# alexpreynolds/starch3

Hardware: AMD Instinct MI355X
Metric: input BED MB/s (cfg2, bzip2 -9, archive bit-identical to CPU starch3 path) (higher is better)
Workload: dtype u8

## Files before the change

starch_amd/csrc/bz2_bwt3.hip:

```cpp
#include "bz2_int.hpp"
#include "bz2_bwt.hpp"

#include <stdio.h>
#include <string.h>

#include <algorithm>
#include <type_traits>
#include <vector>

namespace bz {
namespace {

constexpr int PT = 256;
constexpr int PTILE = 32768;
constexpr int PDIG = 12;
constexpr int PNB = 1 << PDIG;
constexpr int PNB_WIDE = 8192;
static_assert(PTILE <= 32768 && PNB_WIDE <= 8192, "k3_scatter_lds packs (digit << 15) | rotation-in-tile");
constexpr int MAXT = (900064 + PTILE - 1) / PTILE;
constexpr uint32_t W_MAX = 64, S1_MAX = 128, S_MAX = 256, M0_MAX = 512, M1_MAX = 1024, M2_MAX = 2048, M3_MAX = 4096;
#ifndef STARCH_L_MIN
#define STARCH_L_MIN 4096
#endif
constexpr uint32_t L_MIN = STARCH_L_MIN;
// ... 76 lines not shown
    BwtScratch scr;
    Lists L;
    uint32_t nb;
    uint32_t lsel;
    uint32_t tsel;
    uint32_t mode;
    uint32_t keysrc;
    uint64_t* kA;
    uint64_t* kB;
    uint8_t* lA;
    uint8_t* lB;
    uint32_t rtext;
    uint32_t* qhead;
    const uint32_t* qseg;
    uint32_t nbins;
    uint32_t sdig;
};

__device__ __forceinline__ int bits_for3(uint32_t x) { return x ? 32 - __clz(x) : 0; }

__device__ __forceinline__ void wave_sync_lds3()
{
    __builtin_amdgcn_fence(__ATOMIC_RELEASE, "wavefront");
    __builtin_amdgcn_wave_barrier();
    __builtin_amdgcn_fence(__ATOMIC_ACQUIRE, "wavefront");
}

__device__ __forceinline__ uint64_t lanemask_lt()
{
    const int lane = threadIdx.x & 63;
    return lane ? (~0ull >> (64 - lane)) : 0ull;
}

#ifndef STARCH_NT
#define STARCH_NT 0
#endif
#ifndef STARCH_W_UNROLL
#define STARCH_W_UNROLL 0
#endif
template <class T>
__device__ __forceinline__ T ld_nt(const T* p)
{
    if constexpr (STARCH_NT != 0) return __builtin_nontemporal_load(p);
    else return *p;
}
template <class T>
__device__ __forceinline__ void st_nt(T* p, T v)
{
    if constexpr (STARCH_NT != 0) __builtin_nontemporal_store(v, p);
    else *p = v;
}

__device__ __forceinline__ void wave_push(uint32_t* ctr, uint64_t* list, bool pred, uint64_t item)
{
    const uint64_t m = __ballot(pred);
    if (!m) return;
    const int leader = __ffsll((unsigned long long)m) - 1;
    const int lane = threadIdx.x & 63;
    uint32_t base = 0;
    if (lane == leader) base = atomicAdd(ctr, (uint32_t)__popcll(m));
    base = __shfl(base, leader, 64);
    if (pred) list[base + __popcll(m & lanemask_lt())] = item;
}

__device__ __forceinline__ int size_class(uint32_t m)
{
    return m <= W_MAX ? 0 : m <= S1_MAX ? 1 : m <= S_MAX ? 2 : m > L_MIN ? 6 : m <= M0_MAX ? 7 : m <= M1_MAX ? 3 : m <= M2_MAX ? 4
         : m <= M3_MAX ? 5 : 6;
}
__device__ __forceinline__ uint64_t* class_list(const Ctx& c, int cls)
{
    return cls == 0 ? c.L.w : cls == 1 ? c.L.s : cls == 2 ? c.L.s2 : cls == 3 ? c.L.m1 : cls == 4 ? c.L.m2
         : cls == 5 ? c.L.m3 : cls == 7 ? c.L.m0 : c.L.l[c.lsel];
}
__device__ __forceinline__ uint32_t* class_ctr(const Ctx& c, int cls)
{
    return c.L.ctr + (cls == 0 ? C_W : cls == 1 ? C_S : cls == 2 ? C_S2 : cls == 3 ? C_M1 : cls == 4 ? C_M2
                      : cls == 5 ? C_M3 : cls == 7 ? C_M0 : C_L0 + c.lsel);
}

__device__ __forceinline__ void wg_classify(const Ctx& c, uint32_t* sh, bool pred, uint32_t slot, uint32_t s,
                                            uint32_t m, uint32_t shift, uint32_t par)
{
    const int cls = pred ? size_class(m) : -1;
// ... 354 lines not shown
                    const uint64_t a = ix == 0 ? w[0] : ix == 1 ? w[1] : w[2];
                    const uint64_t nx = ix == 0 ? w[1] : ix == 1 ? w[2] : w[3];
                    d[u] = top_digit((a << pb) | ((nx >> 1) >> (63u - pb)), geo);
                }
            }
#pragma unroll
            for (int u = 0; u < SU; ++u) {
                const uint32_t q = q0 + u;
                p[u] = q < e ? atomicAdd(&cur[d[u]], 1u) : 0u;
            }
#pragma unroll
            for (int u = 0; u < SU; ++u) {
                const uint32_t q = q0 + u;
                if (q < e) {
                    const uint32_t r = t0 + q;
                    SA[p[u]] = r;
                    if (tot[d[u]] == 1u) {
                        c.scr.LL[so + p[u]] = (uint8_t)pss_bits(pss, (uint64_t)(r ? r - 1u : n - 1u) * B, B);
                        if (r == 0) c.blocks[b].orig_ptr = p[u];
                    }
                }
            }
        }
        __syncthreads();
    }
}

template <int NB, bool MAT>
__global__ void __launch_bounds__(SCT) k3_scatter_lds(Ctx c)
{
    constexpr uint32_t SH_HALF = NB == PNB ? PTILE / 2 : PTILE / 4;
    constexpr int SU = (int)(SH_HALF / SCT);
    constexpr int BPT = NB / SCT;
    __shared__ uint32_t cur[NB], tot[NB], lst[NB + 1];
    __shared__ uint32_t stage[SH_HALF];
    __shared__ uint8_t stage8[MAT ? 4 : SH_HALF];
    __shared__ uint32_t scan_sh[SCT / 64 + 1];
    __shared__ uint32_t qs[8];
    __shared__ uint32_t job_sh;
    constexpr uint32_t PWN = MAT ? (SH_HALF + 1) * 8 / 64 + 4 : 1;
    __shared__ uint64_t pw[PWN];
    constexpr bool mat = MAT;
    const int tid = threadIdx.x;
    const uint32_t x = xcc_id();
    if (tid < 8) qs[tid] = ((uint32_t)tid < c.nb ? (c.nb - tid + 7) / 8 : 0u) * MAXT;
    __syncthreads();
    for (;;) {
        const uint32_t job = wg_pop(c, qs, &job_sh, x);
        if (job == 0xFFFFFFFFu) break;
        const uint32_t y = job >> 28, k = job & 0x0FFFFFFFu;
        const uint32_t slot = y + 8u * (k / MAXT), tile = k % MAXT;
        const uint32_t b = c.b0 + slot;
        const uint32_t n = c.blocks[b].n;
        const uint32_t t0 = tile * PTILE;
        if (t0 >= n) continue;
        const uint64_t so = (uint64_t)slot * c.scr.stride;
        const uint32_t* th = tile_hist(c, slot);
        for (int i = tid; i < NB; i += SCT) { cur[i] = th[(uint64_t)tile * NB + i]; tot[i] = th[(uint64_t)MAXT * NB + i]; }
        const Geo geo = c.L.geo[slot];
        const uint32_t B = geo.B;
        const uint64_t* pss = c.scr.K + so;
        uint32_t* SA = c.scr.SA + so;
        uint64_t* KM = c.kA + so;
        uint8_t* LS = c.lA ? c.lA + so : nullptr;
        const uint32_t e = n - t0 < (uint32_t)PTILE ? n - t0 : (uint32_t)PTILE;
        for (uint32_t h0 = 0; h0 < e; h0 += SH_HALF) {
            const uint32_t he = e - h0 < SH_HALF ? e - h0 : SH_HALF;
            for (int i = tid; i < NB; i += SCT) lst[i] = 0;
            const uint32_t rs = t0 + h0;
            const uint64_t wbase = rs ? ((uint64_t)(rs - 1) * B) >> 6 : 0;
            if constexpr (mat) {
                const uint64_t wend = (((uint64_t)(rs + he) * B + 64) >> 6) + 2;
                for (uint64_t w = wbase + tid; w < wend; w += SCT) pw[w - wbase] = pss[w];
            }
            __syncthreads();
            const uint32_t q0 = tid * SU;
            uint32_t d[SU], p[SU];
            uint8_t sd[SU];
            {
                const uint64_t bit0 = (uint64_t)(t0 + h0 + q0) * B;
                const uint64_t qw = bit0 >> 6;
                const uint32_t p0 = (uint32_t)(bit0 & 63u);
                const uint64_t w[4] = {pss[qw], pss[qw + 1], pss[qw + 2], pss[qw + 3]};
                const uint32_t sds = 64u - geo.SH - 8u;
#pragma unroll
                for (int u = 0; u < SU; ++u) {
                    const uint32_t bit = p0 + (uint32_t)u * B;
                    const uint32_t ix = bit >> 6, pb = bit & 63u;
                    const uint64_t a = ix == 0 ? w[0] : ix == 1 ? w[1] : w[2];
                    const uint64_t nx = ix == 0 ? w[1] : ix == 1 ? w[2] : w[3];
                    const uint64_t v = (a << pb) | ((nx >> 1) >> (63u - pb));
                    d[u] = top_digit(v, geo);
                    sd[u] = (uint8_t)(v >> sds);
                }
            }
#pragma unroll
            for (int u = 0; u < SU; ++u) p[u] = (q0 + u < he) ? atomicAdd(&lst[d[u]], 1u) : 0u;
            __syncthreads();
            {
                uint32_t v[BPT], sum = 0;
#pragma unroll
                for (int q = 0; q < BPT; ++q) { v[q] = lst[tid * BPT + q]; sum += v[q]; }
                uint32_t run = block_excl_scan_add<uint32_t>(sum, scan_sh, (uint32_t*)nullptr);
#pragma unroll
                for (int q = 0; q < BPT; ++q) { lst[tid * BPT + q] = run; run += v[q]; }
                if (tid == SCT - 1) lst[NB] = run;
            }
            __syncthreads();
#pragma unroll
            for (int u = 0; u < SU; ++u)
                if (q0 + u < he) {
                    const uint32_t j = lst[d[u]] + p[u];
                    stage[j] = (d[u] << 15) | (h0 + q0 + u);
                    if constexpr (!MAT) stage8[j] = sd[u];
                }
            __syncthreads();
            for (uint32_t j = tid; j < he; j += SCT) {
                const uint32_t v = stage[j];
                const uint32_t dg = v >> 15, r = t0 + (v & 0x7FFFu);
                const uint32_t pos = cur[dg] + (j - lst[dg]);
                st_nt(SA + pos, r);
                uint32_t ls = 0;
                if (mat && r) {
                    const uint64_t bit = (uint64_t)(r - 1) * B - (wbase << 6);
                    const uint32_t q = (uint32_t)(bit >> 6), p = (uint32_t)(bit & 63u);
                    ls = (uint32_t)(((pw[q] << p) | ((pw[q + 1] >> 1) >> (63u - p))) >> (64u - B));
                } else if (mat || tot[dg] == 1u) {
                    ls = (uint32_t)pss_bits(pss, (uint64_t)(r ? r - 1u : n - 1u) * B, B);
                }
                if (mat) {
                    const uint64_t bit = (uint64_t)r * B - (wbase << 6);
                    const uint32_t q = (uint32_t)(bit >> 6), p = (uint32_t)(bit & 63u);
                    KM[pos] = ((pw[q] << p) | ((pw[q + 1] >> 1) >> (63u - p))) >> (64u - geo.KB);
                    LS[pos] = (uint8_t)ls;
                }
                if (tot[dg] == 1u) {
                    c.scr.LL[so + pos] = (uint8_t)ls;
                    if (r == 0) c.blocks[b].orig_ptr = pos;
                } else if (!mat && tot[dg] > L_MIN) {
                    c.scr.LL[so + pos] = stage8[j];
                }
            }
            __syncthreads();
            for (int i = tid; i < NB; i += SCT) cur[i] += lst[i + 1] - lst[i];
            __syncthreads();
        }
    }
}

constexpr uint32_t BIN_CH = 4096;
constexpr uint32_t BIN_MAXWG = 128;

__device__ __forceinline__ uint32_t bin_of(uint64_t it, uint32_t i, uint32_t vs)
{
    return (it_slot(it) << vs) | ((i >> 6) & ((1u << vs) - 1u));
}

__global__ void __launch_bounds__(256) k3_bin_hist(const uint64_t* __restrict__ in, uint32_t n, uint32_t nb,
                                                    uint32_t ch, uint32_t* __restrict__ hist,
                                                    uint32_t* __restrict__ colsum, uint32_t vs)
{
    __shared__ uint32_t h[4096];
    for (uint32_t i = threadIdx.x; i < nb; i += 256) h[i] = 0;
    __syncthreads();
    const uint32_t a = blockIdx.x * ch, e = a + ch < n ? a + ch : n;
    for (uint32_t i0 = a; i0 < e; i0 += 256) {
        const uint32_t i = i0 + threadIdx.x;
        const bool ok = i < e;
        const uint32_t b = ok ? bin_of(in[i], i, vs) : 0u;
        const uint64_t act = __ballot(ok);
        if (!act) continue;
        const int lead = __ffsll((unsigned long long)act) - 1;
        const uint32_t b0 = (uint32_t)__shfl((int)b, lead, 64);
        if (__ballot(ok && b == b0) == act) {
            if ((int)(threadIdx.x & 63) == lead) atomicAdd(&h[b0], (uint32_t)__popcll(act));
        } else if (ok) {
            atomicAdd(&h[b], 1u);
        }
    }
// ... 123 lines not shown
        uint8_t* dl = DBL && ks.l ? (par ? c.lA : c.lB) + base : nullptr;
        uint32_t* SA = c.scr.SA + base;
        uint32_t* RK = c.scr.RK + so;
        const uint32_t db = shift < 8 ? shift : 8;
        const uint32_t sh2 = shift - db;
        const uint64_t dmask = (1ull << db) - 1ull;
        const uint8_t* sdig = nullptr;
        if (!DBL && c.sdig && c.rtext == 0 && !c.mode && par == 0 && db == 8) {
            const Geo g = c.L.geo[slot];
            if (shift == g.KB - g.SH) sdig = c.scr.LL + base;
        }
        for (int i = tid; i < LW * 256; i += LT) (&wh[0][0])[i] = 0;
        if (tid == 0) big[256] = 0;
        __syncthreads();
        PLT(t1);
        PLA(0, t0, t1);
#ifndef STARCH_PART_PU
#define STARCH_PART_PU 24
#endif
        constexpr int PU = STARCH_PART_PU;
        for (uint32_t i0 = 0; i0 < m; i0 += PU * LT) {
            uint32_t d[PU];
            if (sdig) {
#pragma unroll
                for (int u = 0; u < PU; ++u) {
                    const uint32_t i = i0 + u * LT + tid;
                    d[u] = sdig[i < m ? i : 0u];
                }
            } else {
                uint32_t vv[PU];
#pragma unroll
                for (int u = 0; u < PU; ++u) {
                    const uint32_t i = i0 + u * LT + tid;
                    vv[u] = ld_nt(sv + (i < m ? i : 0u));
                }
#pragma unroll
                for (int u = 0; u < PU; ++u) {
                    const uint32_t i = i0 + u * LT + tid;
                    d[u] = (uint32_t)((elem_key<DBL>(ks, s + (i < m ? i : 0u), vv[u]) >> sh2) & dmask);
                }
            }
#pragma unroll
            for (int u = 0; u < PU; ++u) {
                const uint32_t i = i0 + u * LT + tid;
                if (!DBL && m <= PL_CAP && i < m) dcache[i] = (uint8_t)d[u];
            }
#pragma unroll
            for (int u = 0; u < PU; ++u)
                if (i0 + u * LT + tid < m) atomicAdd(&wh[wid][d[u]], 1u);
        }
        __syncthreads();
        PLT(t2);
        PLA(1, t1, t2);
        uint32_t tcount = 0;
        if (tid < 256) for (int w = 0; w < LW; ++w) tcount += wh[w][tid];
        const uint32_t pre = block_excl_scan_add<uint32_t>(tid < 256 ? tcount : 0u, scan_sh, (uint32_t*)nullptr);
        if (tid < 256) { st[tid] = pre; cur[tid] = pre; cntd[tid] = tcount; }
        __syncthreads();
        PLT(t3);
        PLA(2, t2, t3);
        const bool staged = !DBL && m <= PL_STG && !(STARCH_PL_STG == 0);
        for (uint32_t i0 = 0; i0 < m; i0 += PU * LT) {
            uint32_t v[PU];
            uint64_t k[PU];
            uint8_t lsy[PU];
#pragma unroll
            for (int u = 0; u < PU; ++u) {
                const uint32_t i = i0 + u * LT + tid;
                v[u] = ld_nt(sv + (i < m ? i : 0u));
            }
            if (!DBL && m <= PL_CAP) {
#pragma unroll
                for (int u = 0; u < PU; ++u) {
                    const uint32_t i = i0 + u * LT + tid;
                    k[u] = (uint64_t)dcache[i < m ? i : 0u] << sh2;
                }
            } else if (sdig) {
#pragma unroll
                for (int u = 0; u < PU; ++u) {
                    const uint32_t i = i0 + u * LT + tid;
                    k[u] = (uint64_t)sdig[i < m ? i : 0u] << sh2;
                }
            } else {
#pragma unroll
                for (int u = 0; u < PU; ++u) {
                    const uint32_t i = i0 + u * LT + tid;
                    k[u] = elem_key<DBL>(ks, s + (i < m ? i : 0u), v[u]);
                }
            }
#pragma unroll
            for (int u = 0; u < PU; ++u) {
                const uint32_t i = i0 + u * LT + tid;
                lsy[u] = dl ? ks.l[s + (i < m ? i : 0u)] : (uint8_t)0;
            }
#pragma unroll
            for (int u = 0; u < PU; ++u) {
                if (i0 + u * LT + tid < m) {
                    const uint32_t p = atomicAdd(&cur[(uint32_t)((k[u] >> sh2) & dmask)], 1u);
                    if (!DBL && staged) stg[p] = v[u];
                    else st_nt(dv + p, v[u]);
                    if constexpr (DBL) dk[p] = k[u];
                    if (dl) dl[p] = lsy[u];
                }
            }
        }
        __syncthreads();
        if (!DBL && staged) {
            for (uint32_t i = tid; i < m; i += LT) st_nt(dv + i, stg[i]);
            __syncthreads();
        }
        PLT(t4);
        PLA(3, t3, t4);
        uint32_t nruns = 0;
        if (tid < 256) {
            const uint32_t cc = cntd[tid], ss = st[tid];
            if (cc == 1) {
                const uint32_t v = dv[ss];
                if (!par) SA[ss] = v;
                c.scr.LL[base + ss] = dl ? dl[ss] : last_sym(c, slot, v);
                if (c.mode) RK[v] = s + ss;
                if (v == 0) c.blocks[b].orig_ptr = s + ss;
                nruns = 1;
            } else if (size_class(cc) == 6 && sh2 == 0) {
                big[atomicAdd(&big[256], 1u)] = tid;
                nruns = 1;
            }
        }
        {
            const uint32_t cc = tid < 256 ? cntd[tid] : 0u;
            const bool push = tid < 256 && cc >= 2 && !(size_class(cc) == 6 && sh2 == 0);
            wg_classify(c, cls_sh, push, slot, s + (tid < 256 ? st[tid] : 0u), cc, sh2, par ^ 1u);
        }
        if (tid < 256) {
            const uint32_t r = wave_reduce_add(nruns);
            if (c.mode && (tid & 63) == 0 && r) atomicAdd(&c.L.runs[slot], r);
        }
        __syncthreads();
        PLT(t5);
        PLA(4, t4, t5);
        const uint32_t nbig = big[256];
        for (uint32_t q = 0; q < nbig; ++q) {
// ... 461 lines not shown
        const uint32_t* info = c.L.hg_info + (uint64_t)q * 512;
        const uint32_t st = info[tid] & ~HG_FINAL;
        const uint32_t en = tid < 255 ? (info[tid + 1] & ~HG_FINAL) : g.m;
        const uint32_t fsz = (info[tid] & HG_FINAL) ? en - st : 0u;
        uint32_t ftot = 0;
        const uint32_t fp = block_excl_scan_add<uint32_t>(fsz, scan_sh, &ftot);
        fin_pre[tid] = fp;
        if (tid == 255) fin_pre[256] = ftot;
        __syncthreads();
        for (uint32_t x = slice * 256u + tid; x < ftot; x += per * 256u) {
            uint32_t lo = 0, hi = 255;
            while (lo < hi) {
                const uint32_t mid = (lo + hi + 1) >> 1;
                if (fin_pre[mid] <= x) lo = mid; else hi = mid - 1;
            }
            const uint32_t b0 = info[lo] & ~HG_FINAL;
            const uint32_t p = b0 + (x - fin_pre[lo]);
            const uint32_t v = dv[p];
            if (!g.par) c.scr.SA[base + p] = v;
            const uint32_t be = lo < 255 ? (info[lo + 1] & ~HG_FINAL) : g.m;
            if (be - b0 == 1) c.scr.LL[base + p] = dl ? dl[p] : last_sym(c, g.slot, v);
            if (c.mode) c.scr.RK[so + v] = g.s + b0;
            if (v == 0) c.blocks[c.b0 + g.slot].orig_ptr = g.s + p;
        }
        __syncthreads();
    }
}

__device__ __forceinline__ void emit_sorted(const Ctx& c, uint32_t slot, uint32_t s, uint32_t j, uint32_t v,
                                            bool valid, uint32_t hp, bool end, uint32_t& runs_acc, uint32_t lsym)
{
    const uint64_t so = (uint64_t)slot * c.scr.stride;
    if (valid) {
        st_nt(c.scr.SA + so + s + j, v);
        st_nt(c.scr.LL + so + s + j, (uint8_t)lsym);
        if (c.mode) c.scr.RK[so + v] = s + hp;
        if (v == 0) c.blocks[c.b0 + slot].orig_ptr = s + j;
    }
    const bool tie = valid && end && j > hp;
    const uint64_t tb = __ballot(tie);
    if (tb) {
        wave_push(c.L.ctr + C_T0 + c.tsel, c.L.t[c.tsel], tie, mk_item(slot, s + hp, j - hp + 1, 0, 0));
        const uint32_t te = wave_reduce_add<uint32_t>(tie ? j - hp + 1 : 0u);
        if ((threadIdx.x & 63) == 0) atomicAdd(c.L.ctr + C_TS0 + c.tsel, te);
    }
    runs_acc += (uint32_t)__popcll(__ballot(valid && end));
}

__device__ __forceinline__ void emit_vals(const Ctx& c, uint32_t slot, uint32_t s, uint32_t j, uint32_t v, bool valid,
                                          uint32_t hp, uint32_t lsym)
{
    if (valid) {
        const uint64_t so = (uint64_t)slot * c.scr.stride;
        st_nt(c.scr.SA + so + s + j, v);
        st_nt(c.scr.LL + so + s + j, (uint8_t)lsym);
        if (c.mode) c.scr.RK[so + v] = s + hp;
        if (v == 0) c.blocks[c.b0 + slot].orig_ptr = s + j;
    }
}

template <int NW>
__device__ __forceinline__ uint32_t tie_reserve(const Ctx& c, uint32_t tcnt, uint32_t* tc, int wid, int lane)
{
    uint32_t* ctr = c.L.ctr + C_T0 + c.tsel;
    if constexpr (NW == 1) {
        uint32_t base = 0;
        if (lane == 0 && tcnt) base = atomicAdd(ctr, tcnt);
        return (uint32_t)__shfl((int)base, 0, 64);
    } else {
        if (lane == 0) tc[wid] = tcnt;
        __syncthreads();
        if (wid == 0 && lane == 0) {
            uint32_t t = 0;
#pragma unroll
            for (int w = 0; w < NW; ++w) t += tc[w];
            tc[NW] = t ? atomicAdd(ctr, t) : 0u;
        }
        __syncthreads();
        uint32_t base = tc[NW];
        for (int w = 0; w < wid; ++w) base += tc[w];
        return base;
    }
}

__device__ __forceinline__ uint64_t shfl64(uint64_t v, uint32_t src)
{
    const uint32_t lo = (uint32_t)__shfl((int)(uint32_t)v, (int)src, 64);
    const uint32_t hi = (uint32_t)__shfl((int)(uint32_t)(v >> 32), (int)src, 64);
// ... 16 lines not shown

template <bool DBL>
__global__ void __launch_bounds__(256) k3_sort_w(Ctx c, const uint64_t* __restrict__ items)
{
    __shared__ uint64_t skey[4][W_MAX + 1];
    __shared__ uint32_t sval[4][W_MAX];
    const uint32_t lane = threadIdx.x & 63, wid = threadIdx.x >> 6;
    const uint32_t xs8 = blockIdx.x & 7u, wseg = (gridDim.x >> 3) * 4u, w_in = (blockIdx.x >> 3) * 4u + wid;
    const uint32_t seg0 = c.qseg[xs8], seg1 = c.qseg[xs8 + 1];
    const uint32_t per_w = (seg1 - seg0 + wseg - 1) / wseg;
    const uint32_t ch = per_w >= 64u ? 64u : (per_w ? per_w : 1u);
    for (uint32_t cb = seg0 + w_in * ch; cb < seg1; cb += wseg * ch) {
        const uint32_t cnt = seg1 - cb < ch ? seg1 - cb : ch;
        const uint64_t myitem = lane < cnt ? items[cb + lane] : 0ull;
        const uint32_t msz = lane < cnt ? it_size(myitem) : 0u;
        for (uint32_t done = 0; done < cnt;) {
            const uint32_t sz = (lane >= done && lane < cnt) ? msz : 0u;
            const uint32_t incl = wave_incl_scan_add(sz);
            const bool take = lane >= done && lane < cnt && incl <= 64u;
            const uint32_t ng = (uint32_t)__popcll(__ballot(take));
            const uint32_t off = incl - sz;
            const uint32_t total = (uint32_t)__shfl((int)incl, (int)(done + ng - 1), 64);
            const uint64_t smask = wave_reduce_or64(take ? (1ull << off) : 0ull);
            const bool valid = lane < total;
            const uint64_t upto = lane == 63 ? ~0ull : ((2ull << lane) - 1ull);
            const uint32_t gi = valid ? done + (uint32_t)__popcll(smask & upto) - 1u : done;
            const uint64_t item = shfl64(myitem, gi);
            const uint32_t goff = (uint32_t)__shfl((int)off, (int)gi, 64);
            const uint32_t gstart = valid ? goff : 0u;
            const uint32_t slot = it_slot(item), s = it_start(item), m = it_size(item), par = it_par(item);
            const uint32_t j = valid ? lane - gstart : 0u;
            const uint32_t* sv = (par ? c.scr.V : c.scr.SA) + (uint64_t)slot * c.scr.stride + s;
            const KeySrc ks = key_src(c, slot, par);
            const uint32_t v = ld_nt(sv + j);
            uint32_t ls;
            uint64_t k = elem_key<DBL>(c, ks, slot, s + j, v, ls);
            if (!valid) k = ~0ull;
            uint32_t r = 0;
            if (ng == 1) {
#if STARCH_W_UNROLL
#pragma unroll 4
#endif
                for (uint32_t q = 0; q < total; ++q) {
                    const uint64_t kq = ((uint64_t)(uint32_t)__builtin_amdgcn_readlane((int)(k >> 32), (int)q) << 32) |
                                        (uint32_t)__builtin_amdgcn_readlane((int)(uint32_t)k, (int)q);
                    r += (kq < k || (kq == k && q < j)) ? 1u : 0u;
                }
            } else {
                const uint32_t maxm = wave_reduce_max(valid ? m : 0u);
#if STARCH_W_UNROLL
#pragma unroll 4
#endif
                for (uint32_t q = 0; q < maxm; ++q) {
                    const bool in = valid && q < m;
                    const uint64_t kq = shfl64(k, in ? gstart + q : lane);
                    r += (in && (kq < k || (kq == k && q < j))) ? 1u : 0u;
                }
            }
            wave_sync_lds3();
            if (valid) { skey[wid][gstart + r] = k; sval[wid][gstart + r] = v | (ls << 24); }
            wave_sync_lds3();
            const uint64_t key = valid ? skey[wid][lane] : 0;
            const uint32_t val = valid ? sval[wid][lane] : 0;
            const bool head = valid && (j == 0 || skey[wid][lane - 1] != key);
            const bool end = valid && (j + 1 == m || skey[wid][lane + 1] != key);
            const uint32_t hp = wave_incl_scan_max<uint32_t>(head ? lane : 0u) - gstart;
            asm volatile("s_waitcnt vmcnt(0)" ::: "memory");
// ... 37 lines not shown

template <int NW>
__device__ __forceinline__ void gsync()
{
    if constexpr (NW == 1) wave_sync_lds3();
    else __syncthreads();
}

template <int E>
struct GrpIn {
    uint64_t item;
    KeySrc ks;
    uint32_t v[E];
    uint32_t v0;
    uint64_t kx[E];
    uint32_t ls[E];
    uint64_t k0;
    uint64_t kb[E];
    uint32_t lb[E];
    uint64_t k0b;
    bool one;
};

template <int NW, int E>
__device__ __forceinline__ void grp_load_vals(const Ctx& c, GrpIn<E>& x, bool ok, int wid, int lane)
{
    if (!ok) x.item = mk_item(0, 0, 1, 0, 0);
    const uint32_t slot = it_slot(x.item), s = it_start(x.item), m = it_size(x.item), par = it_par(x.item);
    const uint32_t* sv = (par ? c.scr.V : c.scr.SA) + (uint64_t)slot * c.scr.stride + s;
    x.ks = key_src(c, slot, par);
#pragma unroll
    for (int e = 0; e < E; ++e) {
        const uint32_t i = (uint32_t)(wid * 64 * E + e * 64 + lane);
        x.v[e] = ld_nt(sv + (i < m ? i : 0u));
    }
    x.v0 = sv[0];
}

__device__ __forceinline__ uint32_t pss_rr(const KeySrc& ks, uint32_t r)
{
    const uint32_t rr = r + ks.off;
    return rr >= ks.n ? rr - ks.n : rr;
}
__device__ __forceinline__ uint32_t pss_pr(const KeySrc& ks, uint32_t r) { return r ? r - 1u : ks.n - 1u; }

#ifndef STARCH_DEFER
#define STARCH_DEFER 1
#endif
template <int NW, bool DBL>
constexpr bool defer_keys() { return !DBL && (STARCH_DEFER == 2 || (STARCH_DEFER == 1 && NW == 1)); }

template <int NW, int E, bool DBL>
__device__ __forceinline__ void grp_load_keys(const Ctx& c, GrpIn<E>& x, int wid, int lane)
{
    const uint32_t s = it_start(x.item), m = it_size(x.item), slot = it_slot(x.item);
    if constexpr (!defer_keys<NW, DBL>()) {
#pragma unroll
        for (int e = 0; e < E; ++e) {
            const uint32_t i = (uint32_t)(wid * 64 * E + e * 64 + lane);
            x.kx[e] = elem_key<DBL>(c, x.ks, slot, s + (i < m ? i : 0u), x.v[e], x.ls[e]);
        }
        x.k0 = elem_key<DBL>(x.ks, s, x.v0);
    } else {
        const uint64_t* __restrict__ w = x.ks.pss;
        const uint32_t* __restrict__ w32 = reinterpret_cast<const uint32_t*>(w);
        const uint32_t B = x.ks.B;
        x.one = x.ks.off == 0 && (B == 1 || B == 2 || B == 4 || B == 5 || B == 6 || B == 8);
// ... 120 lines not shown
    constexpr int DB = CAP <= 128 ? 7 : (CAP <= 256 ? 8 : (CAP <= 1024 ? 10 : (CAP == 2048 ? STARCH_M2_DB : 11)));
    constexpr int NBIN = 1 << DB;
    constexpr int T = NW * 64;
    constexpr int BPT = NBIN / T;
#ifndef STARCH_LIM_NUM
#define STARCH_LIM_NUM 256
#endif
#ifndef STARCH_LIM2_NUM
#define STARCH_LIM2_NUM 512
#endif
    constexpr uint32_t LIMIT = STARCH_LIM_NUM / E;
    __shared__ uint64_t xk_all[IPW][CAP];
    __shared__ uint32_t vb_all[IPW][CAP];
    __shared__ uint16_t bst_all[IPW][NBIN + 2];
    constexpr int UR = NBIN > 256 * NW ? NBIN : 256 * NW;
    __shared__ uint32_t ur_all[IPW][UR];
    __shared__ uint32_t sc_all[IPW][NW + 1];
    constexpr int NB2 = NW == 1 ? 256 : 1024;
    constexpr uint32_t LIMIT2 = STARCH_LIM2_NUM / E;
    __shared__ uint32_t c2_all[IPW][NB2 + 1];
    __shared__ uint32_t sc2_all[IPW][NW + 1];
    __shared__ uint64_t red_all[NWV];
    __shared__ uint32_t wmax_all[NWV];
    __shared__ uint32_t flag_all[NWV];
    __shared__ uint32_t tc_all[NW + 1 > 5 ? NW + 1 : 5];
    uint32_t tacc = 0;
    const int tid = threadIdx.x, lane = tid & 63, wave = tid >> 6;
    const int g = wave / NW, wid = wave % NW, w0 = g * NW;
    uint64_t* xk = xk_all[g];
    uint32_t* wcnt = ur_all[g] + wid * 256;
    uint32_t* sc = sc_all[g];
    const uint64_t lt = lanemask_lt();
    constexpr uint32_t NONE = 0xFFFFFFFFu;
    __shared__ uint32_t qs[8];
    __shared__ uint32_t job_sh;
    const uint32_t xs = xcc_id();
    if (!hard_n) load_qsizes_binned(c, qs);
    const uint32_t nwk = gridDim.x * (uint32_t)IPW;
    const uint32_t e_end = hard_n ? *hard_n : 0u;
    WaveQueue<1> wq;
    uint32_t it_s = blockIdx.x * (uint32_t)IPW + (uint32_t)g;
#ifndef STARCH_LDS_DYN
#define STARCH_LDS_DYN 0
#endif
    const uint32_t xs8 = blockIdx.x & 7u;
    const uint32_t s_end = hard_n ? e_end : c.qseg[xs8 + 1];
    const uint32_t s_nwk = hard_n ? nwk : (gridDim.x >> 3) * (uint32_t)IPW;
    if (!hard_n) it_s = c.qseg[xs8] + (blockIdx.x >> 3) * (uint32_t)IPW + (uint32_t)g;
    auto next_item = [&]() -> uint32_t {
        if (hard_n || !STARCH_LDS_DYN) {
            const uint32_t r = it_s < s_end ? it_s : NONE;
            it_s += s_nwk;
            return r;
        }
        if constexpr (NW == 1) {
            return wq.next(c.qhead, qs, c.qseg, xs);
        } else {
            const uint32_t j = wg_pop(c, qs, &job_sh, xs);
            return j == NONE ? NONE : c.qseg[j >> 28] + (j & 0x0FFFFFFFu);
        }
    };
    uint32_t it = next_item();
    uint32_t it1 = it != NONE ? next_item() : NONE;
    GrpIn<E> cur, nxt;
    cur.item = it != NONE ? items[it] : 0ull;
    grp_load_vals<NW, E>(c, cur, it != NONE, wid, lane);
    grp_load_keys<NW, E, DBL>(c, cur, wid, lane);
    nxt.item = it1 != NONE ? items[it1] : 0ull;
    grp_load_vals<NW, E>(c, nxt, it1 != NONE, wid, lane);
#ifdef STARCH_SORT_PROF
    uint64_t pacc[8] = {0, 0, 0, 0, 0, 0, 0, 0};
#endif
    while (it != NONE) {
    SPROF(t0);
    const uint64_t item = cur.item;
    const uint32_t slot = it_slot(item), s = it_start(item), m = it_size(item);
    grp_finish_keys<NW, E, DBL>(cur);
    gsync<NW>();

    uint64_t k[E];
    uint64_t diff = 0;
#pragma unroll
    for (int e = 0; e < E; ++e) {
        const uint32_t i = (uint32_t)(wid * 64 * E + e * 64 + lane);
        if (i < m) {
            diff |= cur.kx[e] ^ cur.k0;
            k[e] = ((cur.kx[e] & KMASK) << IDXB) | i;
            vb_all[g][i] = cur.v[e] | (cur.ls[e] << 24);
        } else {
            k[e] = ~0ull;
        }
    }
    grp_load_keys<NW, E, DBL>(c, nxt, wid, lane);
// ... 1230 lines not shown
            }
            if (n2) {
                bin(c.L.m2, n2, bout);
                hipLaunchKernelGGL((k3_sort_lds<M2W, M2E, D>), gm2, dim3(64 * M2W), 0, st, c, bout, nullptr);
                sstat("M2");
            }
            if (n0) {
                bin(c.L.m0, n0, bout);
#ifdef STARCH_M0_1W
                static const dim3 gm0w = resident(reinterpret_cast<const void*>(&k3_sort_grp<1, 8, D>));
                clear_h();
                hipLaunchKernelGGL((k3_sort_grp<1, 8, D>), gm0w, dim3(256), 0, st, c, bout, c.L.m0);
                hipLaunchKernelGGL((k3_sort_lds<1, 8, D>), dim3(ncu / 2), dim3(256), 0, st, c, c.L.m0, hard_n);
#else
                hipLaunchKernelGGL((k3_sort_lds<4, 2, D>), gm0, dim3(256), 0, st, c, bout, nullptr);
#endif
                sstat("M0");
            }
            if (n1) {
                bin(c.L.m1, n1, bout);
                hipLaunchKernelGGL((k3_sort_lds<4, 4, D>), gm1, dim3(256), 0, st, c, bout, nullptr);
                sstat("M1");
            }
            if (ns) {
                bin(c.L.s, ns, bout);
                clear_h();
                hipLaunchKernelGGL((k3_sort_grp<1, 2, D>), gs, dim3(256), 0, st, c, bout, c.L.s);
                sstat("S");
                hipLaunchKernelGGL((k3_sort_lds<1, 2, D>), dim3(ncu / 2), dim3(256), 0, st, c, c.L.s, hard_n);
                sstat("S-hard");
            }
            if (ns2) {
                bin(c.L.s2, ns2, bout);
#ifdef STARCH_S2_LDS
                static const dim3 gs2l = resident(reinterpret_cast<const void*>(&k3_sort_lds<4, 1, D>));
                hipLaunchKernelGGL((k3_sort_lds<4, 1, D>), gs2l, dim3(256), 0, st, c, bout, nullptr);
                sstat("S2");
#else
                clear_h();
                hipLaunchKernelGGL((k3_sort_grp<1, 4, D>), gs2, dim3(256), 0, st, c, bout, c.L.s2);
                sstat("S2");
                hipLaunchKernelGGL((k3_sort_lds<1, 4, D>), dim3(ncu / 2), dim3(256), 0, st, c, c.L.s2, hard_n);
                sstat("S2-hard");
#endif
            }
            if (nw) {
                bin(c.L.w, nw, bout);
                hipLaunchKernelGGL(k3_sort_w<D>, gw, dim3(256), 0, st, c, bout);
                sstat("W");
            }
        };
        if (c.keysrc) leaf(std::true_type{});
        else leaf(std::false_type{});
        HIP_CHECK(hipGetLastError());
        zero((0x3Full << C_W) | bit(C_M0));
    };

    static const bool direct = [] { const char* e = getenv("STARCH_SCATTER"); return e && !strcmp(e, "direct"); }();
    const bool kgather = bwt_kgather() && scr.KM0 && !direct;
    if (bwt_kmat() && scr.KM0 && !direct) {
        c.keysrc = 1;
        c.kA = scr.KM0;
        c.kB = scr.KM1;
        c.lA = scr.LS0;
        c.lB = scr.LS1;
    }
    {
        const uint32_t maxw = (uint32_t)pss_words(scr.stride);
        hipLaunchKernelGGL(k3_pss, dim3((maxw + 255) / 256, nb), dim3(256), 0, st, c);
        if (wide) {
            hipLaunchKernelGGL(k3_hist<PNB_WIDE>, dim3(MAXT, nb), dim3(PT), 0, st, c);
            hipLaunchKernelGGL(k3_scan<PNB_WIDE>, dim3(nb), dim3(ST), 0, st, c);
        } else {
            hipLaunchKernelGGL(k3_hist<PNB>, dim3(MAXT, nb), dim3(PT), 0, st, c);
            hipLaunchKernelGGL(k3_scan<PNB>, dim3(nb), dim3(ST), 0, st, c);
        }
        uint32_t* head;
// ... 105 lines not shown
```

Measured before the change: 83810.

## Restructure LDS scatter kernel: prefetch next tile, register cursors, packed bin flags

Reworks the k3_scatter_lds kernel. Per-bin cursors now stay in registers, loaded as uint4 rows, instead of in shared cur/tot arrays. A packed ent[] table encodes each bin's base offset together with singleton and large-bucket flags, which removes the tot[] lookups and the cursor-update pass. The next job is popped during the last half-tile and its histogram row and first key words are prefetched before the scatter loop, overlapping the queue pop and loads with current work. Several barriers are dropped, the scatter loop is batched four at a time, and the unused nontemporal and dynamic-queue compile-time options are removed (they defaulted off). The cost is more register pressure and more complex synchronisation.

```diff
diff --git a/starch_amd/csrc/bz2_bwt3.hip b/starch_amd/csrc/bz2_bwt3.hip
--- a/starch_amd/csrc/bz2_bwt3.hip
+++ b/starch_amd/csrc/bz2_bwt3.hip
@@ -132,24 +132,9 @@
     return lane ? (~0ull >> (64 - lane)) : 0ull;
 }
 
-#ifndef STARCH_NT
-#define STARCH_NT 0
-#endif
 #ifndef STARCH_W_UNROLL
 #define STARCH_W_UNROLL 0
 #endif
-template <class T>
-__device__ __forceinline__ T ld_nt(const T* p)
-{
-    if constexpr (STARCH_NT != 0) return __builtin_nontemporal_load(p);
-    else return *p;
-}
-template <class T>
-__device__ __forceinline__ void st_nt(T* p, T v)
-{
-    if constexpr (STARCH_NT != 0) __builtin_nontemporal_store(v, p);
-    else *p = v;
-}
 
 __device__ __forceinline__ void wave_push(uint32_t* ctr, uint64_t* list, bool pred, uint64_t item)
 {
@@ -570,79 +555,137 @@
     constexpr uint32_t SH_HALF = NB == PNB ? PTILE / 2 : PTILE / 4;
     constexpr int SU = (int)(SH_HALF / SCT);
     constexpr int BPT = NB / SCT;
-    __shared__ uint32_t cur[NB], tot[NB], lst[NB + 1];
+    constexpr uint32_t NONE = 0xFFFFFFFFu;
+    constexpr uint32_t PMASK = (1u << RBITS) - 1u;
+    constexpr uint32_t F_ONE = 1u << 30, F_L = 1u << 31;
+    static_assert(BPT % 4 == 0 && BPT * 2 <= 32, "cursor rows load as uint4; two flag bits per owned bin");
+    __shared__ uint32_t lst[NB];
+    __shared__ uint32_t ent[NB];
     __shared__ uint32_t stage[SH_HALF];
-    __shared__ uint8_t stage8[MAT ? 4 : SH_HALF];
-    __shared__ uint32_t scan_sh[SCT / 64 + 1];
+    __shared__ __attribute__((aligned(16))) uint8_t stage8[MAT ? 16 : SH_HALF];
+    __shared__ uint32_t scan_sh[SCT / 64];
     __shared__ uint32_t qs[8];
     __shared__ uint32_t job_sh;
     constexpr uint32_t PWN = MAT ? (SH_HALF + 1) * 8 / 64 + 4 : 1;
     __shared__ uint64_t pw[PWN];
     constexpr bool mat = MAT;
-    const int tid = threadIdx.x;
+    const int tid = threadIdx.x, lane = tid & 63, wid = tid >> 6;
     const uint32_t x = xcc_id();
     if (tid < 8) qs[tid] = ((uint32_t)tid < c.nb ? (c.nb - tid + 7) / 8 : 0u) * MAXT;
+    for (int i = tid; i < NB; i += SCT) lst[i] = 0;
     __syncthreads();
-    for (;;) {
-        const uint32_t job = wg_pop(c, qs, &job_sh, x);
-        if (job == 0xFFFFFFFFu) break;
+    uint32_t job = wg_pop(c, qs, &job_sh, x);
+    uint32_t curv[BPT];
+    uint64_t w0[4];
+    bool pre = false;
+    uint32_t flv = 0, fslot = NONE;
+    auto load_row = [&](const uint32_t* th, uint32_t tile) {
+        const uint4* row = reinterpret_cast<const uint4*>(th + (uint64_t)tile * NB + tid * BPT);
+#pragma unroll
+        for (int q = 0; q < BPT / 4; ++q) {
+            const uint4 v = row[q];
+            curv[4 * q] = v.x; curv[4 * q + 1] = v.y; curv[4 * q + 2] = v.z; curv[4 * q + 3] = v.w;
+        }
+    };
+    auto load_w0 = [&](const uint64_t* pss, uint32_t t0, uint32_t B) {
+        const uint64_t qw = ((uint64_t)(t0 + tid * SU) * B) >> 6;
+#pragma unroll
+        for (int q = 0; q < 4; ++q) w0[q] = pss[qw + q];
+    };
+    while (job != NONE) {
         const uint32_t y = job >> 28, k = job & 0x0FFFFFFFu;
         const uint32_t slot = y + 8u * (k / MAXT), tile = k % MAXT;
         const uint32_t b = c.b0 + slot;
         const uint32_t n = c.blocks[b].n;
         const uint32_t t0 = tile * PTILE;
-        if (t0 >= n) continue;
+        if (t0 >= n) {
+            job = wg_pop(c, qs, &job_sh, x);
+            pre = false;
+            continue;
+        }
         const uint64_t so = (uint64_t)slot * c.scr.stride;
         const uint32_t* th = tile_hist(c, slot);
-        for (int i = tid; i < NB; i += SCT) { cur[i] = th[(uint64_t)tile * NB + i]; tot[i] = th[(uint64_t)MAXT * NB + i]; }
         const Geo geo = c.L.geo[slot];
         const uint32_t B = geo.B;
         const uint64_t* pss = c.scr.K + so;
         uint32_t* SA = c.scr.SA + so;
+        uint8_t* LL = c.scr.LL + so;
         uint64_t* KM = c.kA + so;
         uint8_t* LS = c.lA ? c.lA + so : nullptr;
+        if (!pre) {
+            load_row(th, tile);
+            load_w0(pss, t0, B);
+        }
+        if (slot != fslot) {
+            const uint32_t* tot = th + (uint64_t)MAXT * NB + tid * BPT;
+            flv = 0;
+#pragma unroll
+            for (int q = 0; q < BPT; ++q) {
+                const uint32_t t = tot[q];
+                flv |= (t == 1u ? 1u : t > L_MIN ? 2u : 0u) << (2 * q);
+            }
+            fslot = slot;
+        }
         const uint32_t e = n - t0 < (uint32_t)PTILE ? n - t0 : (uint32_t)PTILE;
+        uint32_t njob = NONE;
+        pre = false;
         for (uint32_t h0 = 0; h0 < e; h0 += SH_HALF) {
             const uint32_t he = e - h0 < SH_HALF ? e - h0 : SH_HALF;
-            for (int i = tid; i < NB; i += SCT) lst[i] = 0;
+            const bool last = h0 + SH_HALF >= e;
             const uint32_t rs = t0 + h0;
             const uint64_t wbase = rs ? ((uint64_t)(rs - 1) * B) >> 6 : 0;
             if constexpr (mat) {
                 const uint64_t wend = (((uint64_t)(rs + he) * B + 64) >> 6) + 2;
                 for (uint64_t w = wbase + tid; w < wend; w += SCT) pw[w - wbase] = pss[w];
             }
-            __syncthreads();
+            if (last && tid == 0) job_sh = xq_pop(c.qhead, qs, x);
             const uint32_t q0 = tid * SU;
             uint32_t d[SU], p[SU];
-            uint8_t sd[SU];
             {
                 const uint64_t bit0 = (uint64_t)(t0 + h0 + q0) * B;
                 const uint64_t qw = bit0 >> 6;
                 const uint32_t p0 = (uint32_t)(bit0 & 63u);
-                const uint64_t w[4] = {pss[qw], pss[qw + 1], pss[qw + 2], pss[qw + 3]};
+                if (h0 != 0) {
+#pragma unroll
+                    for (int q = 0; q < 4; ++q) w0[q] = pss[qw + q];
+                }
                 const uint32_t sds = 64u - geo.SH - 8u;
+                uint32_t sdw[SU / 4] = {};
 #pragma unroll
                 for (int u = 0; u < SU; ++u) {
                     const uint32_t bit = p0 + (uint32_t)u * B;
                     const uint32_t ix = bit >> 6, pb = bit & 63u;
-                    const uint64_t a = ix == 0 ? w[0] : ix == 1 ? w[1] : w[2];
-                    const uint64_t nx = ix == 0 ? w[1] : ix == 1 ? w[2] : w[3];
+                    const uint64_t a = ix == 0 ? w0[0] : ix == 1 ? w0[1] : w0[2];
+                    const uint64_t nx = ix == 0 ? w0[1] : ix == 1 ? w0[2] : w0[3];
                     const uint64_t v = (a << pb) | ((nx >> 1) >> (63u - pb));
                     d[u] = top_digit(v, geo);
-                    sd[u] = (uint8_t)(v >> sds);
+                    sdw[u / 4] |= ((uint32_t)(v >> sds) & 0xFFu) << (8 * (u % 4));
+                }
+                if constexpr (!MAT) {
+                    uint32_t* s8 = reinterpret_cast<uint32_t*>(stage8 + q0);
+#pragma unroll
+                    for (int q = 0; q < SU / 4; ++q) s8[q] = sdw[q];
                 }
             }
 #pragma unroll
             for (int u = 0; u < SU; ++u) p[u] = (q0 + u < he) ? atomicAdd(&lst[d[u]], 1u) : 0u;
             __syncthreads();
+            if (last) njob = job_sh;
             {
                 uint32_t v[BPT], sum = 0;
 #pragma unroll
                 for (int q = 0; q < BPT; ++q) { v[q] = lst[tid * BPT + q]; sum += v[q]; }
-                uint32_t run = block_excl_scan_add<uint32_t>(sum, scan_sh, (uint32_t*)nullptr);
-#pragma unroll
-                for (int q = 0; q < BPT; ++q) { lst[tid * BPT + q] = run; run += v[q]; }
-                if (tid == SCT - 1) lst[NB] = run;
+                const uint32_t inc = wave_incl_scan_add(sum);
+                if (lane == 63) scan_sh[wid] = inc;
+                __syncthreads();
+                uint32_t run = wave_reduce_add<uint32_t>(lane < wid ? scan_sh[lane] : 0u) + inc - sum;
+#pragma unroll
+                for (int q = 0; q < BPT; ++q) {
+                    lst[tid * BPT + q] = run;
+                    ent[tid * BPT + q] = ((curv[q] - run) & PMASK) | (((flv >> (2 * q)) & 3u) << 30);
+                    curv[q] += v[q];
+                    run += v[q];
+                }
             }
             __syncthreads();
 #pragma unroll
@@ -650,20 +693,43 @@
                 if (q0 + u < he) {
                     const uint32_t j = lst[d[u]] + p[u];
                     stage[j] = (d[u] << 15) | (h0 + q0 + u);
-                    if constexpr (!MAT) stage8[j] = sd[u];
                 }
             __syncthreads();
-            for (uint32_t j = tid; j < he; j += SCT) {
-                const uint32_t v = stage[j];
-                const uint32_t dg = v >> 15, r = t0 + (v & 0x7FFFu);
-                const uint32_t pos = cur[dg] + (j - lst[dg]);
-                st_nt(SA + pos, r);
+#pragma unroll
+            for (int q = 0; q < BPT; ++q) lst[tid * BPT + q] = 0;
+            if (njob != NONE) {
+                const uint32_t nk = njob & 0x0FFFFFFFu;
+                const uint32_t nslot = (njob >> 28) + 8u * (nk / MAXT), ntile = nk % MAXT;
+                if (ntile * (uint32_t)PTILE < c.blocks[c.b0 + nslot].n) {
+                    load_row(tile_hist(c, nslot), ntile);
+                    load_w0(c.scr.K + (uint64_t)nslot * c.scr.stride, ntile * (uint32_t)PTILE, c.L.geo[nslot].B);
+                    pre = true;
+                }
+            }
+            for (int u0 = 0; u0 < SU && (uint32_t)tid + (uint32_t)u0 * SCT < he; u0 += 4) {
+                uint32_t sv[4], se[4];
+#pragma unroll
+                for (int i = 0; i < 4; ++i) {
+                    const uint32_t j = (uint32_t)tid + (uint32_t)(u0 + i) * SCT;
+                    sv[i] = stage[j < he ? j : (uint32_t)tid];
+                }
+#pragma unroll
+                for (int i = 0; i < 4; ++i) se[i] = ent[sv[i] >> 15];
+#pragma unroll
+                for (int i = 0; i < 4; ++i) {
+                const uint32_t j = (uint32_t)tid + (uint32_t)(u0 + i) * SCT;
+                if (j >= he) break;
+                const uint32_t v = sv[i];
+                const uint32_t r = t0 + (v & 0x7FFFu);
+                const uint32_t en = se[i];
+                const uint32_t pos = (en + j) & PMASK;
+                SA[pos] = r;
                 uint32_t ls = 0;
                 if (mat && r) {
                     const uint64_t bit = (uint64_t)(r - 1) * B - (wbase << 6);
                     const uint32_t q = (uint32_t)(bit >> 6), p = (uint32_t)(bit & 63u);
                     ls = (uint32_t)(((pw[q] << p) | ((pw[q + 1] >> 1) >> (63u - p))) >> (64u - B));
-                } else if (mat || tot[dg] == 1u) {
+                } else if (mat || (en & F_ONE)) {
                     ls = (uint32_t)pss_bits(pss, (uint64_t)(r ? r - 1u : n - 1u) * B, B);
                 }
                 if (mat) {
@@ -672,17 +738,17 @@
                     KM[pos] = ((pw[q] << p) | ((pw[q + 1] >> 1) >> (63u - p))) >> (64u - geo.KB);
                     LS[pos] = (uint8_t)ls;
                 }
-                if (tot[dg] == 1u) {
-                    c.scr.LL[so + pos] = (uint8_t)ls;
+                if (en & F_ONE) {
+                    LL[pos] = (uint8_t)ls;
                     if (r == 0) c.blocks[b].orig_ptr = pos;
-                } else if (!mat && tot[dg] > L_MIN) {
-                    c.scr.LL[so + pos] = stage8[j];
+                } else if (!mat && (en & F_L)) {
+                    LL[pos] = stage8[(v & 0x7FFFu) - h0];
                 }
+                }
             }
             __syncthreads();
-            for (int i = tid; i < NB; i += SCT) cur[i] += lst[i + 1] - lst[i];
-            __syncthreads();
-        }
+        }
+        job = njob;
     }
 }
 
@@ -872,7 +938,7 @@
 #pragma unroll
                 for (int u = 0; u < PU; ++u) {
                     const uint32_t i = i0 + u * LT + tid;
-                    vv[u] = ld_nt(sv + (i < m ? i : 0u));
+                    vv[u] = sv[i < m ? i : 0u];
                 }
 #pragma unroll
                 for (int u = 0; u < PU; ++u) {
@@ -907,7 +973,7 @@
 #pragma unroll
             for (int u = 0; u < PU; ++u) {
                 const uint32_t i = i0 + u * LT + tid;
-                v[u] = ld_nt(sv + (i < m ? i : 0u));
+                v[u] = sv[i < m ? i : 0u];
             }
             if (!DBL && m <= PL_CAP) {
 #pragma unroll
@@ -938,7 +1004,7 @@
                 if (i0 + u * LT + tid < m) {
                     const uint32_t p = atomicAdd(&cur[(uint32_t)((k[u] >> sh2) & dmask)], 1u);
                     if (!DBL && staged) stg[p] = v[u];
-                    else st_nt(dv + p, v[u]);
+                    else dv[p] = v[u];
                     if constexpr (DBL) dk[p] = k[u];
                     if (dl) dl[p] = lsy[u];
                 }
@@ -946,7 +1012,7 @@
         }
         __syncthreads();
         if (!DBL && staged) {
-            for (uint32_t i = tid; i < m; i += LT) st_nt(dv + i, stg[i]);
+            for (uint32_t i = tid; i < m; i += LT) dv[i] = stg[i];
             __syncthreads();
         }
         PLT(t4);
@@ -1474,8 +1540,8 @@
 {
     const uint64_t so = (uint64_t)slot * c.scr.stride;
     if (valid) {
-        st_nt(c.scr.SA + so + s + j, v);
-        st_nt(c.scr.LL + so + s + j, (uint8_t)lsym);
+        c.scr.SA[so + s + j] = v;
+        c.scr.LL[so + s + j] = (uint8_t)lsym;
         if (c.mode) c.scr.RK[so + v] = s + hp;
         if (v == 0) c.blocks[c.b0 + slot].orig_ptr = s + j;
     }
@@ -1494,8 +1560,8 @@
 {
     if (valid) {
         const uint64_t so = (uint64_t)slot * c.scr.stride;
-        st_nt(c.scr.SA + so + s + j, v);
-        st_nt(c.scr.LL + so + s + j, (uint8_t)lsym);
+        c.scr.SA[so + s + j] = v;
+        c.scr.LL[so + s + j] = (uint8_t)lsym;
         if (c.mode) c.scr.RK[so + v] = s + hp;
         if (v == 0) c.blocks[c.b0 + slot].orig_ptr = s + j;
     }
@@ -1578,7 +1644,7 @@
             const uint32_t j = valid ? lane - gstart : 0u;
             const uint32_t* sv = (par ? c.scr.V : c.scr.SA) + (uint64_t)slot * c.scr.stride + s;
             const KeySrc ks = key_src(c, slot, par);
-            const uint32_t v = ld_nt(sv + j);
+            const uint32_t v = sv[j];
             uint32_t ls;
             uint64_t k = elem_key<DBL>(c, ks, slot, s + j, v, ls);
             if (!valid) k = ~0ull;
@@ -1682,7 +1748,7 @@
 #pragma unroll
     for (int e = 0; e < E; ++e) {
         const uint32_t i = (uint32_t)(wid * 64 * E + e * 64 + lane);
-        x.v[e] = ld_nt(sv + (i < m ? i : 0u));
+        x.v[e] = sv[i < m ? i : 0u];
     }
     x.v0 = sv[0];
 }
@@ -1869,33 +1935,17 @@
     uint32_t* sc = sc_all[g];
     const uint64_t lt = lanemask_lt();
     constexpr uint32_t NONE = 0xFFFFFFFFu;
-    __shared__ uint32_t qs[8];
-    __shared__ uint32_t job_sh;
-    const uint32_t xs = xcc_id();
-    if (!hard_n) load_qsizes_binned(c, qs);
     const uint32_t nwk = gridDim.x * (uint32_t)IPW;
     const uint32_t e_end = hard_n ? *hard_n : 0u;
-    WaveQueue<1> wq;
     uint32_t it_s = blockIdx.x * (uint32_t)IPW + (uint32_t)g;
-#ifndef STARCH_LDS_DYN
-#define STARCH_LDS_DYN 0
-#endif
     const uint32_t xs8 = blockIdx.x & 7u;
     const uint32_t s_end = hard_n ? e_end : c.qseg[xs8 + 1];
     const uint32_t s_nwk = hard_n ? nwk : (gridDim.x >> 3) * (uint32_t)IPW;
     if (!hard_n) it_s = c.qseg[xs8] + (blockIdx.x >> 3) * (uint32_t)IPW + (uint32_t)g;
     auto next_item = [&]() -> uint32_t {
-        if (hard_n || !STARCH_LDS_DYN) {
-            const uint32_t r = it_s < s_end ? it_s : NONE;
-            it_s += s_nwk;
-            return r;
-        }
-        if constexpr (NW == 1) {
-            return wq.next(c.qhead, qs, c.qseg, xs);
-        } else {
-            const uint32_t j = wg_pop(c, qs, &job_sh, xs);
-            return j == NONE ? NONE : c.qseg[j >> 28] + (j & 0x0FFFFFFFu);
-        }
+        const uint32_t r = it_s < s_end ? it_s : NONE;
+        it_s += s_nwk;
+        return r;
     };
     uint32_t it = next_item();
     uint32_t it1 = it != NONE ? next_item() : NONE;
@@ -3192,17 +3242,11 @@
             }
             if (ns2) {
                 bin(c.L.s2, ns2, bout);
-#ifdef STARCH_S2_LDS
-                static const dim3 gs2l = resident(reinterpret_cast<const void*>(&k3_sort_lds<4, 1, D>));
-                hipLaunchKernelGGL((k3_sort_lds<4, 1, D>), gs2l, dim3(256), 0, st, c, bout, nullptr);
-                sstat("S2");
-#else
                 clear_h();
                 hipLaunchKernelGGL((k3_sort_grp<1, 4, D>), gs2, dim3(256), 0, st, c, bout, c.L.s2);
                 sstat("S2");
                 hipLaunchKernelGGL((k3_sort_lds<1, 4, D>), dim3(ncu / 2), dim3(256), 0, st, c, c.L.s2, hard_n);
                 sstat("S2-hard");
-#endif
             }
             if (nw) {
                 bin(c.L.w, nw, bout);
```

Result: faster. 85650 (median of 6 runs) (+2.2%).
